# sleep3r/crispy

Hardware: AMD Instinct MI355X
Metric: concurrent real-time 48 kHz streams/GPU (RNNoise) (higher is better)
Workload: dtype f32; 1 GPU; Batched RNNoise: 4096 concurrent 48 kHz mono streams per GPU x 100 frames per step (BASELINE configs[1]), seeded synthetic int8 weights; streams_per_gpu=4096, output_finite=True

## Files before the change

crispy_amd/csrc/rn_kernels.hip:

```cpp
#include <type_traits>
#include "rn_common.h"
#include "rn_wave_sums.h"

namespace crispy {
namespace {

constexpr int WAVE = 64;

#ifdef RN_PROFILE
#define RN_PROF_DECL long long tprev_ = clock64(); \
  float* profp_ = (DBG && a.dbg) ? a.dbg + (long)blockIdx.x * RN_DBG_FLOATS + 3824 : nullptr;
#define STAMP(k) { const long long tn_ = clock64(); if (profp_ && threadIdx.x == 0) profp_[k] += (float)(tn_ - tprev_); tprev_ = tn_; }
#elif defined(RN_STOP_AFTER)
#define RN_PROF_DECL
#define STAMP(k) { if ((k) == RN_STOP_AFTER) { __syncthreads(); continue; } }
#else
#define RN_PROF_DECL
#define STAMP(k)
#endif

__device__ __constant__ int c_second_check[16] = {0, 0, 3, 2, 3, 2, 5, 2, 3, 2, 3, 2, 5, 2, 3, 2};

__device__ __forceinline__ float2 cmul(float2 a, float2 b) {
  return make_float2(a.x * b.x - a.y * b.y, a.x * b.y + a.y * b.x);
}
__device__ __forceinline__ float2 cadd(float2 a, float2 b) { return make_float2(a.x + b.x, a.y + b.y); }
__device__ __forceinline__ float2 csub(float2 a, float2 b) { return make_float2(a.x - b.x, a.y - b.y); }
__device__ __forceinline__ float2 cconj(float2 a) { return make_float2(a.x, -a.y); }

template <int CTRL, int ROW_MASK = 0xf>
__device__ __forceinline__ float dpp_mov(float v) {
  const int iv = __float_as_int(v);
  return __int_as_float(__builtin_amdgcn_update_dpp(0, iv, CTRL, ROW_MASK, 0xf, false));
}
template <int CTRL>
__device__ __forceinline__ float dpp_add(float v) {
  float r = v + dpp_mov<CTRL>(v);
  asm volatile("" : "+v"(r));
  return r;
}
template <class V>
__device__ __forceinline__ void lane_put(V& v, V s, int l) {
  static_assert(sizeof(V) == 4, "one dword");
  asm("v_writelane_b32 %0, %1, %2" : "+v"(v) : "s"(s), "n"(l));
}
template <class T>
__device__ __forceinline__ T ld_u32(const T* __restrict__ base, unsigned idx) {
  return *reinterpret_cast<const T*>(reinterpret_cast<const char*>(base) + idx * (unsigned)sizeof(T));
}
__device__ __forceinline__ float wave_sum(float v) {
  v += dpp_mov<0xB1>(v);
  v += dpp_mov<0x4E>(v);
  v += dpp_mov<0x141>(v);
  v += dpp_mov<0x140>(v);
  v += dpp_mov<0x142, 0xa>(v);
  v += dpp_mov<0x143, 0xc>(v);
  return __int_as_float(__builtin_amdgcn_readlane(__float_as_int(v), 63));
}

template <int NW>
__device__ __forceinline__ void rn_sync() {
  if constexpr (NW == 1) {
    __syncthreads();
  } else {
    __builtin_amdgcn_fence(__ATOMIC_RELEASE, "wavefront");
    __builtin_amdgcn_s_waitcnt(0xc07f);
    __builtin_amdgcn_wave_barrier();
    __builtin_amdgcn_fence(__ATOMIC_ACQUIRE, "wavefront");
  }
}

template <int R>
__device__ __forceinline__ void butterfly(const float2 (&v)[R], float2 (&o)[R]);

template <>
__device__ __forceinline__ void butterfly<4>(const float2 (&v)[4], float2 (&o)[4]) {
  const float2 s0 = cadd(v[0], v[2]), d0 = csub(v[0], v[2]);
  const float2 s1 = cadd(v[1], v[3]), d1 = csub(v[1], v[3]);
  o[0] = cadd(s0, s1);
  o[2] = csub(s0, s1);
  o[1] = make_float2(d0.x + d1.y, d0.y - d1.x);
  o[3] = make_float2(d0.x - d1.y, d0.y + d1.x);
}
template <>
// ... 318 lines not shown
      const int pidx = lane + WAVE * m;
      if (pidx < 200 && (lane & 1) == 0) { part[pidx >> 1] = clo[m]; part[100 + (pidx >> 1)] = chi[m]; }
    }
    band_total(Cout);
    if (XE) {
#pragma unroll
      for (int m = 0; m < 4; ++m) {
        const int pidx = lane + WAVE * m;
        if (pidx < 200 && (lane & 1) == 0) { part[pidx >> 1] = xlo[m]; part[100 + (pidx >> 1)] = xhi[m]; }
      }
      band_total(Xout);
    }
  }
}

struct TansigTab {
  float t[4];
  __device__ __forceinline__ void load(const float* __restrict__ table, int lane) {
#pragma unroll
    for (int q = 0; q < 4; ++q) t[q] = ld_u32(table, (unsigned)min(64 * q + lane, 200));
  }
  __device__ __forceinline__ float at(int i) const {
    const int addr = (i & 63) << 2;
    const float v0 = __int_as_float(__builtin_amdgcn_ds_bpermute(addr, __float_as_int(t[0])));
    const float v1 = __int_as_float(__builtin_amdgcn_ds_bpermute(addr, __float_as_int(t[1])));
    const float v2 = __int_as_float(__builtin_amdgcn_ds_bpermute(addr, __float_as_int(t[2])));
    const float v3 = __int_as_float(__builtin_amdgcn_ds_bpermute(addr, __float_as_int(t[3])));
    const int q = i >> 6;
    return q == 0 ? v0 : (q == 1 ? v1 : (q == 2 ? v2 : v3));
  }
};
__device__ __forceinline__ float tansig_approx(float x, const TansigTab& table) {
#pragma clang fp contract(off)
  const float x0 = x;
  float sign = 1.f;
  if (x < 0.f) { x = -x; sign = -1.f; }
  x = fminf(x, 8.f);
  const int i = (int)floorf(.5f + 25.f * x);
  x = x - .04f * (float)i;
  float y = table.at(i);
  const float dy = 1.f - y * y;
  y = y + (x * dy) * (1.f - y * x);
  y = sign * y;
  if (!(x0 > -8.f)) y = -1.f;
  if (!(x0 < 8.f)) y = 1.f;
  return y;
}
__device__ __forceinline__ float sigmoid_approx(float x, const TansigTab& table) {
  return .5f + .5f * tansig_approx(.5f * x, table);
}

typedef _Float16 h8 __attribute__((ext_vector_type(8)));
#define RN_LANE_RANGE(site) __builtin_assume((unsigned)lane < (unsigned)WAVE)
constexpr int RN_BLK3 = 1, RN_BLK2 = 1, RN_BLK1 = 4;

typedef unsigned int rn_u4 __attribute__((ext_vector_type(4)));
__device__ __forceinline__ float dot_vad(__amdgpu_buffer_rsrc_t rs, int w_off, const float* x, float acc0) {
  float acc = acc0, acc1 = 0.f;
#pragma unroll
  for (int k = 0; k < 3; ++k) {
    const h8 w = __builtin_bit_cast(h8, __builtin_amdgcn_raw_buffer_load_b128(rs, 0, (w_off + k) * 16, 0));
#pragma unroll
    for (int e = 0; e < 8; e += 2) {
      acc = fmaf((float)w[e], x[8 * k + e], acc);
      acc1 = fmaf((float)w[e + 1], x[8 * k + e + 1], acc1);
    }
  }
  return acc + acc1;
}

typedef int rn_i4 __attribute__((ext_vector_type(4)));
constexpr int RN_IMG8_LD = 144;
__device__ __forceinline__ float wave_max(float v) {
  unsigned u = __float_as_uint(v);
  auto dm = [](unsigned x, auto ctrl) {
    return (unsigned)__builtin_amdgcn_update_dpp(0, (int)x, decltype(ctrl)::value, 0xf, 0xf, false);
  };
  u = max(u, dm(u, std::integral_constant<int, 0xB1>{}));
  u = max(u, dm(u, std::integral_constant<int, 0x4E>{}));
  u = max(u, dm(u, std::integral_constant<int, 0x141>{}));
  u = max(u, dm(u, std::integral_constant<int, 0x140>{}));
  unsigned m = (unsigned)__builtin_amdgcn_readlane((int)u, 0);
  m = max(m, (unsigned)__builtin_amdgcn_readlane((int)u, 16));
  m = max(m, (unsigned)__builtin_amdgcn_readlane((int)u, 32));
  m = max(m, (unsigned)__builtin_amdgcn_readlane((int)u, 48));
  return __uint_as_float(m);
}
struct RnScale { float up, dn; };
__device__ __forceinline__ RnScale scale_of(float m) {
  int eb = (__float_as_int(m) >> 23) & 0xff;
  eb = min(max(eb, 64), 250);
  RnScale r;
  r.up = __int_as_float((283 - eb) << 23);
  r.dn = __int_as_float((eb - 29) << 23);
  return r;
}
__device__ __forceinline__ void digits_store(signed char* img, int i, float v, float up) {
  const int q = __float2int_rn(v * up);
  const unsigned r = ((unsigned)q + 0x00808080u) ^ 0x00808080u;
  img[i] = (signed char)(r & 0xff);
  img[RN_IMG8_LD + i] = (signed char)((r >> 8) & 0xff);
  img[2 * RN_IMG8_LD + i] = (signed char)((r >> 16) & 0xff);
  img[3 * RN_IMG8_LD + i] = (signed char)(r >> 24);
}
template <int NPAD, class F>
__device__ __forceinline__ RnScale image_i8(signed char* img, int lane, F f) {
  constexpr int NT = (NPAD + WAVE - 1) / WAVE;
  float v[NT];
  float m = 0.f;
#pragma unroll
  for (int j = 0; j < NT; ++j) {
    const int i = lane + WAVE * j;
    v[j] = i < NPAD ? f(min(i, NPAD - 1)) : 0.f;
    m = __uint_as_float(max(__float_as_uint(m), __float_as_uint(v[j]) & 0x7fffffffu));
  }
  const RnScale sc = scale_of(wave_max(m));
#pragma unroll
  for (int j = 0; j < NT; ++j) {
    const int i = lane + WAVE * j;
    if (i < NPAD) digits_store(img, i, v[j], sc.up);
  }
  return sc;
}
__device__ __forceinline__ rn_u4 wload8(__amdgpu_buffer_rsrc_t rs, int row16, int off16) {
  return __builtin_amdgcn_raw_buffer_load_b128(rs, row16, off16 * 16, 0);
}
template <int MK16, int NK16, int ROWS, int NR>
__device__ __forceinline__ void dotn_i(__amdgpu_buffer_rsrc_t rs, int w_off, int u_off, const int (&row)[NR],
                                       const signed char* xa, const signed char* xb, int toff, float sa, float sb,
                                       float (&acc)[NR]) {
  constexpr int K16 = MK16 + NK16;
  constexpr int BLK = NR >= 3 ? RN_BLK3 : (NR == 2 ? RN_BLK2 : RN_BLK1);
  constexpr int NBLK = (K16 + BLK - 1) / BLK;
  constexpr int NC = NR >= 3 ? 1 : 2;
  int row16[NR];
#pragma unroll
  for (int r = 0; r < NR; ++r) row16[r] = row[r] * 16;
  asm volatile("" : "+v"(toff));
  const rn_u4* xa4 = reinterpret_cast<const rn_u4*>(xa + toff);
  const rn_u4* xb4 = reinterpret_cast<const rn_u4*>(xb + toff);
  rn_u4 w[2][BLK][NR];
  rn_u4 xc = MK16 > 0 ? xa4[0] : xb4[0], xn = xc;
#pragma unroll
  for (int q = 0; q < BLK; ++q)
    if (q < K16) {
#pragma unroll
      for (int r = 0; r < NR; ++r)
        w[0][q][r] = wload8(rs, row16[r], q < MK16 ? w_off + q * ROWS : u_off + (q - MK16) * ROWS);
    }
  rn_i4 a4[NR][NC];
#pragma unroll
  for (int r = 0; r < NR; ++r)
#pragma unroll
    for (int c = 0; c < NC; ++c) a4[r][c] = rn_i4{0, 0, 0, 0};
  auto fold = [&](float s) {
#pragma unroll
    for (int r = 0; r < NR; ++r) {
      rn_i4 d = a4[r][0];
      if (NC == 2) d += a4[r][1];
      float f = (float)d[0] * s;
      f = fmaf((float)d[1], s * 256.f, f);
      f = fmaf((float)d[2], s * 65536.f, f);
      f = fmaf((float)d[3], s * 16777216.f, f);
      acc[r] += f;
#pragma unroll
      for (int c = 0; c < NC; ++c) a4[r][c] = rn_i4{0, 0, 0, 0};
    }
  };
#pragma unroll
  for (int blk = 0; blk < NBLK; ++blk) {
    if (blk + 1 < NBLK) {
#pragma unroll
      for (int q = 0; q < BLK; ++q) {
        const int k = (blk + 1) * BLK + q;
        if (k < K16) {
#pragma unroll
          for (int r = 0; r < NR; ++r)
            w[(blk + 1) & 1][q][r] = wload8(rs, row16[r], k < MK16 ? w_off + k * ROWS : u_off + (k - MK16) * ROWS);
        }
      }
    }
    __builtin_amdgcn_sched_barrier(0);
#pragma unroll
    for (int q = 0; q < BLK; ++q) {
      const int k = blk * BLK + q;
      if (k < K16) {
        if (k + 1 < K16) xn = k + 1 < MK16 ? xa4[k + 1] : xb4[k + 1 - MK16];
        if (MK16 > 0 && NK16 > 0 && k == MK16) fold(sa);
        if (!(k == 0 || (MK16 > 0 && NK16 > 0 && k == MK16))) {
#pragma unroll
          for (int r = 0; r < NR; ++r)
#pragma unroll
            for (int c = 0; c < NC; ++c) asm volatile("" : "+v"(a4[r][c]));
        }
        __builtin_amdgcn_sched_barrier(0);
#pragma unroll
        for (int e = 0; e < 4; ++e) {
#pragma unroll
          for (int r = 0; r < NR; ++r)
            a4[r][e % NC] = __builtin_amdgcn_mfma_i32_4x4x4i8((int)xc[e], (int)w[blk & 1][q][r][e], a4[r][e % NC], 0, 0, 0);
        }
        __builtin_amdgcn_sched_barrier(0);
        xc = xn;
      }
    }
  }
  fold(NK16 > 0 ? sb : sa);
}
template <int K16, int ROWS>
__device__ __forceinline__ float dot_i(__amdgpu_buffer_rsrc_t rs, int w_off, int row, const signed char* x, int toff,
                                       float s, float acc0) {
  const int rows[1] = {row};
  float acc[1] = {acc0};
  dotn_i<K16, 0, ROWS, 1>(rs, w_off, w_off, rows, x, x, toff, s, s, acc);
  return acc[0];
}
template <int NW, int M, int N>
__device__ __forceinline__ void gru_layer_i(__amdgpu_buffer_rsrc_t rs, int w_off, int u_off,
                                            const float* __restrict__ bias, const signed char* in_img, float sin,
                                            float* state, float* zbuf, signed char* st_img, int toff,
                                            const TansigTab& tansig, int lane) {
  constexpr int ROWS = 3 * N;
  constexpr int MK16 = (M + 15) / 16, NK16 = (N + 15) / 16;
  constexpr int NRZ = (2 * N + WAVE - 1) / WAVE, NRC = (N + WAVE - 1) / WAVE;
  const float S = 1.f / 256.f;
  const RnScale sst = image_i8<NK16 * 16>(st_img, lane, [&](int i) { return i < N ? state[min(i, N - 1)] : 0.f; });
  rn_sync<NW>();
  {
    int rows[NRZ];
    float acc[NRZ];
#pragma unroll
    for (int r = 0; r < NRZ; ++r) {
      rows[r] = min(lane + WAVE * r, 2 * N - 1);
      acc[r] = ld_u32(bias, (unsigned)rows[r]);
    }
    dotn_i<MK16, NK16, ROWS, NRZ>(rs, w_off, u_off, rows, in_img, st_img, toff, sin, sst.dn, acc);
#pragma unroll
    for (int r = 0; r < NRZ; ++r) {
      const int row = lane + WAVE * r;
      const float s = sigmoid_approx(S * acc[r], tansig);
      if (row < 2 * N) {
        if (row < N) zbuf[row] = s;
        else digits_store(st_img, row - N, state[row - N] * s, sst.up);
      }
    }
  }
  rn_sync<NW>();
  {
    int rows[NRC];
    float acc[NRC];
#pragma unroll
    for (int r = 0; r < NRC; ++r) {
      rows[r] = 2 * N + min(lane + WAVE * r, N - 1);
      acc[r] = ld_u32(bias, (unsigned)rows[r]);
    }
    dotn_i<MK16, NK16, ROWS, NRC>(rs, w_off, u_off, rows, in_img, st_img, toff, sin, sst.dn, acc);
#pragma unroll
    for (int r = 0; r < NRC; ++r) {
      const int i = lane + WAVE * r;
      if (i < N) {
        float c = S * acc[r];
        c = c < 0.f ? 0.f : c;
        const float z = zbuf[i];
        state[i] = z * state[i] + (1.f - z) * c;
      }
    }
  }
  rn_sync<NW>();
}

struct alignas(16) RnSlot {
  float2 A[482];
  float2 Bb[482];
  float U[200];
  float Ex[24], Ep[24], Exp[24];
  int pitch_index;
  float pitch_gain;
  int silence;
  int pad;
};
template <int NW> struct RnLdsT;
template <> struct alignas(16) RnLdsT<1> {
  RnSlot s[1];
  float ceps[8 * 22];
  float rnn_state[168];
};
template <> struct alignas(16) RnLdsT<3> {
  RnSlot s[2];
  float2 pa[482];
  float2 pb[482];
  float ceps[8 * 22];
  float rnn_state[168];
  int pitch_index[2];
  float pitch_gain[2];
};
static_assert(sizeof(RnLdsT<1>) <= 10240, "16 workgroups per CU need <= 10 KB of LDS each");
static_assert(6 * sizeof(RnLdsT<3>) <= 160 * 1024, "six stage-pipelined streams per CU");

constexpr int U_G = 0, U_R = 24, U_VAD = 46, U_LY = 48;
constexpr int PL_FEAT = 800, PL_Z = 842, PL_DENSE = 938, PL_A_FREE = 800, PL_U_FREE = 48;

struct Cand {
  float num, den;
  int idx;
};
__device__ __forceinline__ bool cand_better(const Cand& a, const Cand& b) {
  const float l = a.num * b.den, r = b.num * a.den;
  return (l > r) || (!(r > l) && a.idx < b.idx);
}
__device__ __forceinline__ Cand wave_best(Cand c) {
#pragma unroll
  for (int off = 32; off > 0; off >>= 1) {
    Cand o;
    o.num = __shfl_xor(c.num, off, WAVE);
    o.den = __shfl_xor(c.den, off, WAVE);
    o.idx = __shfl_xor(c.idx, off, WAVE);
    if (cand_better(o, c)) c = o;
  }
  c.num = __shfl(c.num, 0, WAVE);
  c.den = __shfl(c.den, 0, WAVE);
  c.idx = __shfl(c.idx, 0, WAVE);
  return c;
}

typedef float rn_f2 __attribute__((ext_vector_type(2)));
__device__ __forceinline__ void lag_window(const float* xr, int lane, float (&xv)[8]) {
#pragma unroll
  for (int m = 0; m < 7; ++m) xv[m] = xr[WAVE * m];
  xv[7] = 0.f;
  if (lane < 32) xv[7] = xr[WAVE * 7];
}
template <int NL, bool SQ>
__device__ __forceinline__ void lag_dots(const float (&xv)[8], const float* const (&yr)[NL], int lane, float (&sxy)[NL],
                                         float (&syy)[NL]) {
#pragma unroll
  for (int q = 0; q < NL; ++q) { sxy[q] = 0.f; syy[q] = 0.f; }
#pragma unroll
  for (int q = 0; q < NL; ++q) {
#pragma unroll
    for (int m = 0; m < 7; ++m) {
      const float y = yr[q][WAVE * m];
      sxy[q] = fmaf(xv[m], y, sxy[q]);
      if (SQ) syy[q] = fmaf(y, y, syy[q]);
    }
  }
  if (lane < 32) {
#pragma unroll
    for (int q = 0; q < NL; ++q) {
      const float y = yr[q][WAVE * 7];
      sxy[q] = fmaf(xv[7], y, sxy[q]);
      if (SQ) syy[q] = fmaf(y, y, syy[q]);
    }
  }
  wave_sums<NL>(sxy);
  if (SQ) wave_sums<NL>(syy);
}

#ifndef RN_POISON_LDS
#define RN_POISON_LDS 0
#endif
[[maybe_unused]] __device__ __forceinline__ void rn_poison_lds(uint32_t* p, int words) {
  for (int i = threadIdx.x; i < words; i += WAVE) p[i] = 0x7fc0dead;
  __syncthreads();
}

__device__ __forceinline__ float2* rn_lds_lp(RnLdsT<1>& L) { return L.s[0].Bb; }
__device__ __forceinline__ float2* rn_lds_sa(RnLdsT<1>& L) { return L.s[0].A; }
__device__ __forceinline__ float2* rn_lds_lp(RnLdsT<3>& L) { return L.pb; }
__device__ __forceinline__ float2* rn_lds_sa(RnLdsT<3>& L) { return L.pa; }

template <bool DBG, int NW>
__device__ __forceinline__ void rn_frame_body(const RnArgs& a) {
  __shared__ RnLdsT<NW> L;
  const int wave = NW == 1 ? 0 : (int)(threadIdx.x >> 6);
  const int lane0 = threadIdx.x & (WAVE - 1);
  const int b = blockIdx.x;
  if (b >= a.B) return;
  int lane = lane0;
  const RnTables* tab = a.tab;
  const float* xs = a.xhp + (long)b * a.xhp_stride;
  if constexpr (NW == 1) {
    unsigned hw;
    asm volatile("s_getreg_b32 %0, hwreg(HW_REG_HW_ID)" : "=s"(hw));
    const unsigned pr = hw & 3u;
    if (pr == 0) __builtin_amdgcn_s_setprio(0);
    else if (pr == 1) __builtin_amdgcn_s_setprio(1);
    else if (pr == 2) __builtin_amdgcn_s_setprio(2);
    else __builtin_amdgcn_s_setprio(3);
  }

#if RN_POISON_LDS
  rn_poison_lds(reinterpret_cast<uint32_t*>(&L), sizeof(L) / 4);
#endif

  const bool own_a = NW == 1 || wave == 0, own_b = NW == 1 || wave == 1, own_c = NW == 1 || wave == 2;
  if (own_b)
    for (int i = lane; i < 176; i += WAVE) L.ceps[i] = a.ceps[(long)b * 176 + i];
  if (own_c)
    for (int i = lane; i < 168; i += WAVE) L.rnn_state[i] = a.rnn[(long)b * 168 + i];
  float2 synth[4];
  float* synth_g = a.synth + (long)b * 480;
#pragma unroll
  for (int m = 0; m < 4; ++m) {
    const int n = lane + WAVE * m;
// ... 120 lines not shown
        float y[14];
  #pragma unroll
        for (int q = 0; q < 14; ++q) {
          float sum = w[q + 5];
          sum = fmaf(lpc2[0], w[q + 4], sum);
          sum = fmaf(lpc2[1], w[q + 3], sum);
          sum = fmaf(lpc2[2], w[q + 2], sum);
          sum = fmaf(lpc2[3], w[q + 1], sum);
          sum = fmaf(lpc2[4], w[q], sum);
          y[q] = sum;
        }
        rn_sync<NW>();
  #pragma unroll
        for (int q = 0; q < 14; ++q)
          if (base + q < 864) lp[base + q] = y[q];
        rn_sync<NW>();
      }
      STAMP(0)
      lane = lane0;
      asm volatile("" : "+v"(lane));
      RN_LANE_RANGE(4);

      float* x4 = Sa;
      float* y4 = Sa + 240;
      float* pre = Sa;
      {
        float vx[4], vy[7];
  #pragma unroll
        for (int m = 0; m < 4; ++m) vx[m] = lp[384 + 2 * min(lane + WAVE * m, 239)];
  #pragma unroll
        for (int m = 0; m < 7; ++m) vy[m] = lp[2 * min(lane + WAVE * m, 386)];
  #pragma unroll
        for (int m = 0; m < 4; ++m) {
          const int j = lane + WAVE * m;
          if (j < 240) x4[j] = vx[m];
        }
  #pragma unroll
        for (int m = 0; m < 7; ++m) {
          const int j = lane + WAVE * m;
          if (j < 392) y4[j] = j < 387 ? vy[m] : 0.f;
        }
      }
      rn_sync<NW>();
      int best0, best1;
      {
        float xc[3] = {0.f, 0.f, 0.f};
        {
          const float4* xv4 = reinterpret_cast<const float4*>(x4);
          const float* yp = y4 + 3 * min(lane, 48);
          float y0 = yp[0], y1 = yp[1];
  #pragma unroll 4
          for (int j4 = 0; j4 < 60; ++j4) {
            const float4 xv = xv4[j4];
            const int j = 4 * j4;
            const float y2 = yp[j + 2], y3 = yp[j + 3], y4v = yp[j + 4], y5 = yp[j + 5];
            xc[0] = fmaf(xv.x, y0, xc[0]);
            xc[1] = fmaf(xv.x, y1, xc[1]);
            xc[2] = fmaf(xv.x, y2, xc[2]);
            xc[0] = fmaf(xv.y, y1, xc[0]);
            xc[1] = fmaf(xv.y, y2, xc[1]);
            xc[2] = fmaf(xv.y, y3, xc[2]);
            xc[0] = fmaf(xv.z, y2, xc[0]);
            xc[1] = fmaf(xv.z, y3, xc[1]);
            xc[2] = fmaf(xv.z, y4v, xc[2]);
            xc[0] = fmaf(xv.w, y3, xc[0]);
            xc[1] = fmaf(xv.w, y4v, xc[1]);
            xc[2] = fmaf(xv.w, y5, xc[2]);
            y0 = y4v;
            y1 = y5;
          }
        }
        STAMP(1)
        {
          float loc[7];
          float run = 0.f;
  #pragma unroll
          for (int q = 0; q < 7; ++q) {
            const int j = 7 * lane + q;
            const float v = j < 392 ? y4[j] : 0.f;
            loc[q] = run;
            run = fmaf(v, v, run);
          }
          float incl = run;
  #pragma unroll
          for (int off = 1; off < WAVE; off <<= 1) {
            const float o = __shfl_up(incl, off, WAVE);
            if (lane >= off) incl += o;
          }
          const float excl = incl - run;
          rn_sync<NW>();
  #pragma unroll
          for (int q = 0; q < 7; ++q)
            if (7 * lane + q < 392) pre[7 * lane + q] = excl + loc[q];
        }
        rn_sync<NW>();
        Cand c0 = {-1.f, 0.f, 1 << 20}, c1 = {-1.f, 0.f, 1 << 20};
        int nvalid = 0;
  #pragma unroll
        for (int rr = 0; rr < 3; ++rr) {
          const int lag = 3 * lane + rr;
          if (lag < 147 && xc[rr] > 0.f) {
            const float syy = fmaxf(1.f, 1.f + (pre[lag + 240] - pre[lag]));
            const float x16 = xc[rr] * 1e-12f;
            const Cand c = {x16 * x16, syy, lag};
            ++nvalid;
            if (cand_better(c, c0)) { c1 = c0; c0 = c; }
            else if (cand_better(c, c1)) c1 = c;
          }
        }
        const int total_valid = __popcll(__ballot(nvalid > 0)) == 0 ? 0 : (int)wave_sum((float)nvalid);
        const Cand w0 = wave_best(c0);
        const Cand mine = (c0.idx == w0.idx) ? c1 : c0;
        const Cand w1 = wave_best(mine);
        if (total_valid == 0) { best0 = 0; best1 = 1; }
        else if (total_valid == 1) { best0 = w0.idx; best1 = 0; }
        else { best0 = w0.idx; best1 = w1.idx; }
      }
      best0 = __builtin_amdgcn_readfirstlane(best0);
      best1 = __builtin_amdgcn_readfirstlane(best1);
      rn_sync<NW>();
      STAMP(2)

      float* fine = Sa;
      float xwin[8];
      for (int i = lane; i < 296; i += WAVE) fine[i] = 0.f;
      rn_sync<NW>();
      {
        const int ca = 2 * min(best0, best1), cb = 2 * max(best0, best1);
        Cand bestc = {-1.f, 0.f, 0};
        bool any = false;
        int lagi[10];
        bool use[10];
        const float* yr[10];
  #pragma unroll
        for (int q = 0; q < 10; ++q) {
          const int pass = q / 5, d = q % 5 - 2;
          const int i = (pass == 0 ? ca : cb) + d;
          use[q] = !(i < 0 || i >= 294) && !(pass == 1 && abs(i - ca) <= 2);
          lagi[q] = use[q] ? i : 0;
          yr[q] = lp + lagi[q] + lane;
        }
        float sxy[10], syy[10];
        lag_window(lp + 384 + lane, lane, xwin);
        lag_dots<10, true>(xwin, yr, lane, sxy, syy);
  #pragma unroll
        for (int q = 0; q < 10; ++q) {
          if (use[q]) {
            const float syq = fmaxf(1.f, 1.f + syy[q]);
            const float xv = fmaxf(-1.f, sxy[q]);
            if (lane == 0) fine[lagi[q]] = xv;
            if (xv > 0.f) {
              const float x16 = xv * 1e-12f;
              const Cand c = {x16 * x16, syq, lagi[q]};
              if (!any || cand_better(c, bestc)) { bestc = c; any = true; }
            }
          }
        }
        rn_sync<NW>();
        const int bp = any ? bestc.idx : 0;
        int offset = 0;
        if (bp > 0 && bp < 293) {
          const float fa = fine[bp - 1], fb = fine[bp], fc = fine[bp + 1];
          if ((fc - fa) > .7f * (fb - fa)) offset = 1;
          else if ((fa - fc) > .7f * (fb - fc)) offset = -1;
        }
        pitch_index = __builtin_amdgcn_readfirstlane(768 - (2 * bp - offset));
      }
      rn_sync<NW>();
      STAMP(3)
      if (DBG && a.dbg && t == a.T - 1) {
        float* D = a.dbg + (long)b * RN_DBG_FLOATS;
        for (int i = lane; i < 864; i += WAVE) D[984 + i] = lp[i];
        if (lane == 0) D[1848] = (float)pitch_index;
  #ifndef RN_PROFILE
        for (int i = lane; i < 480; i += WAVE) D[3824 + i] = xw[480 + i];
  #endif
      }

      {
        const float* x = lp + 384;
        int T0 = pitch_index / 2;
        const int prev_period = last_period / 2;
        if (T0 >= 384) T0 = 383;
        int T = T0;
        float xx, xy;
        {
          const float* yr[2] = {x + lane, x - T0 + lane};
          float sa[2], sb[2];
          lag_dots<2, false>(xwin, yr, lane, sa, sb);
          xx = sa[0];
          xy = sa[1];
        }
        float* yyl = Sa + 296;
        {
          float loc[6];
          float run = 0.f;
  #pragma unroll
          for (int q = 0; q < 6; ++q) {
            const int m = 6 * lane + 1 + q;
            const float u = x[-m], v = x[480 - m];
            run += u * u - v * v;
            loc[q] = run;
          }
          float incl = run;
  #pragma unroll
          for (int off = 1; off < WAVE; off <<= 1) {
            const float o = __shfl_up(incl, off, WAVE);
            if (lane >= off) incl += o;
          }
          const float excl = incl - run;
  #pragma unroll
          for (int q = 0; q < 6; ++q) yyl[6 * lane + 1 + q] = fmaxf(0.f, xx + (excl + loc[q]));
          if (lane == 0) yyl[0] = xx;
        }
        rn_sync<NW>();
        float yy = yyl[T0];
        float best_xy = xy, best_yy = yy;
        const float g0 = xy / sqrtf(1.f + xx * yy);
        float g = g0;
        int t1v = 0, t1bv = 0;
        float xya = 0.f, xyb = 0.f;
        static_assert((2 * 383 + 14) / (2 * 14) < 30, "candidates k >= 14 are out of range for every T0");
  #pragma unroll
        for (int c = 0; c < 3; ++c) {
          const int k0 = 2 + 4 * c;
          if ((2 * T0 + k0) / (2 * k0) >= 30) {
            constexpr int NKC = 4;
            const float* yr[2 * NKC];
            int t1[NKC], t1b[NKC];
  #pragma unroll
            for (int q = 0; q < NKC; ++q) {
              const int k = k0 + q;
              t1[q] = 0; t1b[q] = 0;
              const int T1 = (2 * T0 + k) / (2 * k);
              if (T1 >= 30) {
                t1[q] = T1;
                if (k == 2) t1b[q] = (T1 + T0 > 384) ? T0 : T0 + T1;
                else t1b[q] = (2 * c_second_check[k] * T0 + k) / (2 * k);
              }
              yr[2 * q] = x - t1[q] + lane;
              yr[2 * q + 1] = x - t1b[q] + lane;
            }
            float sa[2 * NKC], sb[2 * NKC];
            lag_dots<2 * NKC, false>(xwin, yr, lane, sa, sb);
  #pragma unroll
            for (int q = 0; q < NKC; ++q) {
              const int l = k0 + q - 2;
              lane_put(t1v, t1[q], l);
              lane_put(t1bv, t1b[q], l);
              lane_put(xya, sa[2 * q], l);
              lane_put(xyb, sa[2 * q + 1], l);
            }
          }
        }
        {
          const int T1 = t1v;
          const float xyk = .5f * (xya + xyb);
          const float yyk = .5f * (yyl[t1v] + yyl[t1bv]);
          const int k = lane + 2;
          const float g1 = xyk / sqrtf(1.f + xx * yyk);
          float cont;
          if (abs(T1 - prev_period) <= 1) cont = last_gain;
          else if (abs(T1 - prev_period) <= 2 && 5 * k * k < T0) cont = .5f * last_gain;
          else cont = 0.f;
          float thresh = fmaxf(.3f, .7f * g0 - cont);
          if (T1 < 90) thresh = fmaxf(.4f, .85f * g0 - cont);
          else if (T1 < 60) thresh = fmaxf(.5f, .9f * g0 - cont);
          const unsigned long long pass = __ballot(lane < 14 && T1 >= 30 && g1 > thresh);
          if (pass != 0ull) {
            const int w = 63 - __builtin_clzll(pass);
            best_xy = __int_as_float(__builtin_amdgcn_readlane(__float_as_int(xyk), w));
            best_yy = __int_as_float(__builtin_amdgcn_readlane(__float_as_int(yyk), w));
            T = __builtin_amdgcn_readlane(T1, w);
            g = __int_as_float(__builtin_amdgcn_readlane(__float_as_int(g1), w));
          }
        }
        best_xy = fmaxf(0.f, best_xy);
        float pgv = (best_yy <= best_xy) ? 1.f : best_xy / (best_yy + 1.f);
        float xc3[3];
        {
          const float* yr[3] = {x - (T - 1) + lane, x - T + lane, x - (T + 1) + lane};
          float sb[3];
          lag_dots<3, false>(xwin, yr, lane, xc3, sb);
        }
        int offset = 0;
        if ((xc3[2] - xc3[0]) > .7f * (xc3[1] - xc3[0])) offset = 1;
        else if ((xc3[0] - xc3[2]) > .7f * (xc3[1] - xc3[2])) offset = -1;
        if (pgv > g) pgv = g;
        pitch_index = 2 * T + offset;
        if (pitch_index < 60) pitch_index = 60;
// ... 82 lines not shown
        }
      }
      {
        if (lane < 6) {
          float v = se * dct_norm;
          if (lane == 0) v -= 1.3f;
          if (lane == 1) v -= 0.9f;
          Rb[KB_FEAT + 34 + lane] = v;
        }
        if (lane == 6) Rb[KB_FEAT + 40] = .01f * (float)(pitch_index - 300);
        silence = E < 0.04f;
        if (!silence && lane < RN_NB) {
          float v = sl * dct_norm;
          if (lane == 0) v -= 12.f;
          if (lane == 1) v -= 4.f;
          Rb[KB_FEAT + lane] = v;
          L.ceps[memid * RN_NB + lane] = v;
        }
      }
      rn_sync<NW>();
      if (silence) {
        if (lane < RN_NFEAT) Rb[KB_FEAT + lane] = 0.f;
        if (lane < RN_NB) SL.U[U_G + lane] = 0.f;
        rn_sync<NW>();
      } else {
        {
          const int m1 = (memid < 1) ? 8 + memid - 1 : memid - 1;
          const int m2 = (memid < 2) ? 8 + memid - 2 : memid - 2;
          if (lane < 6) {
            const float c0 = L.ceps[memid * RN_NB + lane];
            const float c1 = L.ceps[m1 * RN_NB + lane];
            const float c2 = L.ceps[m2 * RN_NB + lane];
            Rb[KB_FEAT + lane] = c0 + c1 + c2;
            Rb[KB_FEAT + RN_NB + lane] = c0 - c2;
            Rb[KB_FEAT + RN_NB + 6 + lane] = c0 - 2.f * c1 + c2;
          }
          memid = (memid + 1 == 8) ? 0 : memid + 1;
        }
        {
          const int ci = lane >> 3, cj = lane & 7;
          float dist = 0.f;
  #pragma unroll
          for (int k = 0; k < RN_NB; ++k) {
            const float d = L.ceps[ci * RN_NB + k] - L.ceps[cj * RN_NB + k];
            dist = fmaf(d, d, dist);
          }
          float md = (ci == cj) ? 1e15f : dist;
          md = fminf(md, dpp_mov<0xB1>(md));
          md = fminf(md, dpp_mov<0x4E>(md));
          md = fminf(md, dpp_mov<0x141>(md));
          const float sv = wave_sum(md) * .125f;
          if (lane == 0) Rb[KB_FEAT + 41] = sv / 8.f - 2.1f;
        }
        rn_sync<NW>();
        STAMP(7)
      }
      if constexpr (NW > 1) {
        if (lane == 0) { SL.pitch_index = pitch_index; SL.pitch_gain = pitch_gain; SL.silence = silence ? 1 : 0; }
      }
    }
    if (own_c) {
      if constexpr (NW > 1) {
        pitch_index = __builtin_amdgcn_readfirstlane(SL.pitch_index);
        pitch_gain = SL.pitch_gain;
        silence = __builtin_amdgcn_readfirstlane(SL.silence) != 0;
      }
      if (!silence) {
        lane = lane0;
        asm volatile("" : "+v"(lane));
        RN_LANE_RANGE(1);
        const float S = 1.f / 256.f;
        float* feat = Rb + KB_FEAT;
        float* dense = Rb + PL_DENSE;
        float* zbuf = Rb + PL_Z;
        TansigTab tansig;
        tansig.load(tab->tansig, lane);
        signed char* in_img = reinterpret_cast<signed char*>(SL.U + PL_U_FREE);
        signed char* st_img = reinterpret_cast<signed char*>(Xf + PL_A_FREE);
        const int toff = (lane & 3) * RN_IMG8_LD;
        RnScale sc = image_i8<48>(in_img, lane, [&](int i) { return i < RN_NFEAT ? feat[i] : 0.f; });
        rn_sync<NW>();
        {
          const int row = min(lane, 23);
          const float acc = dot_i<rn_k16(42), 24>(wrs, RnPack8::ID_W, row, in_img, toff, sc.dn, wpf[RnPack::ID_B + row]);
          const float d = tansig_approx(S * acc, tansig);
          if (lane < 24) dense[lane] = d;
        }
        rn_sync<NW>();
        sc = image_i8<32>(in_img, lane, [&](int i) { return i < 24 ? dense[i] : 0.f; });
        gru_layer_i<NW, 24, 24>(wrs, RnPack8::VG_W, RnPack8::VG_R, wpf + RnPack::VG_B, in_img, sc.dn,
                            L.rnn_state, zbuf, st_img, toff, tansig, lane);
        {
          float acc = 0.f;
          if (lane == 0) {
            acc = wpf[RnPack::VO_B];
            acc = dot_vad(wrs, RnPack::VO_W, L.rnn_state, acc);
          }
          const float v = sigmoid_approx(S * acc, tansig);
          if (lane == 0) SL.U[U_VAD] = v;
        }
        sc = image_i8<96>(in_img, lane, [&](int i) {
          return i < 24 ? dense[i] : (i < 48 ? L.rnn_state[i - 24] : (i < 90 ? feat[i - 48] : 0.f)); });
        rn_sync<NW>();
        vad_prob = SL.U[U_VAD];
        STAMP(8)
        gru_layer_i<NW, 90, 48>(wrs, RnPack8::NG_W, RnPack8::NG_R, wpf + RnPack::NG_B, in_img, sc.dn,
                            L.rnn_state + 24, zbuf, st_img, toff, tansig, lane);
        STAMP(9)
        sc = image_i8<128>(in_img, lane, [&](int i) { return i < 72 ? L.rnn_state[i] : (i < 114 ? feat[i - 72] : 0.f); });
        rn_sync<NW>();
        gru_layer_i<NW, 114, 96>(wrs, RnPack8::DG_W, RnPack8::DG_R, wpf + RnPack::DG_B, in_img, sc.dn,
                             L.rnn_state + 72, zbuf, st_img, toff, tansig, lane);
        sc = image_i8<96>(st_img, lane, [&](int i) { return L.rnn_state[72 + i]; });
        rn_sync<NW>();
        {
          const int row = min(lane, RN_NB - 1);
          const float acc = dot_i<rn_k16(96), RN_NB>(wrs, RnPack8::DO_W, row, st_img, toff, sc.dn, wpf[RnPack::DO_B + row]);
          const float gv = sigmoid_approx(S * acc, tansig);
          if (lane < RN_NB) SL.U[U_G + lane] = gv;
        }
        rn_sync<NW>();
        STAMP(10)

        lane = lane0;
        asm volatile("" : "+v"(lane));
        RN_LANE_RANGE(2);
        float2 fq[4];
        int bq[4];
        {
          float4 pq[4];
  #pragma unroll
          for (int m = 0; m < 4; ++m) {
            const unsigned pidx = (unsigned)min(lane + WAVE * m, 199);
            pq[m] = *reinterpret_cast<const float4*>(SL.Bb + 2 * pidx);
            fq[m] = ld_u32(reinterpret_cast<const float2*>(tab->bin_frac), pidx);
            bq[m] = ld_u32(tab->bin_band, 2 * pidx);
          }
          if (lane < RN_NB) {
            const float ex = SL.Exp[lane], gg = SL.U[U_G + lane];
            float r;
            if (ex > gg) r = 1.f;
            else r = (ex * ex) * (1.f - gg * gg) / (.001f + (gg * gg) * (1.f - ex * ex));
            r = sqrtf(fminf(1.f, fmaxf(0.f, r)));
            r *= sqrtf(SL.Ex[lane] / (1e-8f + SL.Ep[lane]));
            SL.U[U_R + lane] = r;
          }
          rn_sync<NW>();
          float* part = Xf + PL_A_FREE;
          float* part_hi = SL.U + PL_U_FREE;
  #pragma unroll
          for (int m = 0; m < 4; ++m) {
            const int pidx = lane + WAVE * m;
            if (pidx < 200) {
              const float r0 = SL.U[U_R + bq[m]], r1 = SL.U[U_R + bq[m] + 1];
              const float rf0 = (1.f - fq[m].x) * r0 + fq[m].x * r1;
              const float rf1 = (1.f - fq[m].y) * r0 + fq[m].y * r1;
              float4 x = *reinterpret_cast<const float4*>(SL.A + 2 * pidx);
              x.x = fmaf(rf0, pq[m].x, x.x);
              x.y = fmaf(rf0, pq[m].y, x.y);
              x.z = fmaf(rf1, pq[m].z, x.z);
              x.w = fmaf(rf1, pq[m].w, x.w);
              *reinterpret_cast<float4*>(SL.A + 2 * pidx) = x;
              float e0 = x.x * x.x; e0 += x.y * x.y;
              float e1 = x.z * x.z; e1 += x.w * x.w;
              float lo = (1.f - fq[m].x) * e0 + (1.f - fq[m].y) * e1;
              float hi = fq[m].x * e0 + fq[m].y * e1;
              lo = dpp_add<0xB1>(lo);
              hi = dpp_add<0xB1>(hi);
              if ((lane & 1) == 0) { part[pidx >> 1] = lo; part_hi[pidx >> 1] = hi; }
            }
          }
        }
        rn_sync<NW>();
        float sum;
        {
          const float* part = Xf + PL_A_FREE;
          const float* part_hi = SL.U + PL_U_FREE;
          sum = band_sum(part, part_hi, be, lane);
        }
        if (lane < RN_NB) {
          SL.U[U_R + lane] = sqrtf(SL.Ex[lane] / (1e-8f + sum));
          const float gg = fmaxf(SL.U[U_G + lane], .6f * lastg);
          SL.U[U_G + lane] = gg;
          lastg = gg;
        }
        rn_sync<NW>();
        float nq[4][2], gq[4][2];
        float4 xq[4];
  #pragma unroll
        for (int m = 0; m < 4; ++m) {
          nq[m][0] = SL.U[U_R + bq[m]]; nq[m][1] = SL.U[U_R + bq[m] + 1];
          gq[m][0] = SL.U[U_G + bq[m]]; gq[m][1] = SL.U[U_G + bq[m] + 1];
          xq[m] = *reinterpret_cast<const float4*>(SL.A + 2 * min(lane + WAVE * m, 199));
        }
  #pragma unroll
        for (int m = 0; m < 4; ++m) {
          const int pidx = lane + WAVE * m;
          if (pidx < 200) {
            const float n0 = nq[m][0], n1 = nq[m][1];
            const float g0 = gq[m][0], g1 = gq[m][1];
// ... 136 lines not shown
```

Measured before the change: 751,800 concurrent real-time 48 kHz streams (whole job).

## Pin scale math to scalar regs, use swizzle/bpermute reductions, branchless candidate select

Moves the quantization scale computation into a header and uses inline asm to keep it in scalar registers. Power-of-two scale multiplies become exponent-bit adds. The candidate argmax reduction is rewritten with ds_bpermute/ds_swizzle, branchless selection and readlane broadcasts, and the prefix scans use bpermute in place of __shfl_up. The number of MFMA accumulator chains is now parameterized by wave count (one chain when NW==1), which cuts accumulator registers but lengthens the dependency chain.

```diff
diff --git a/crispy_amd/csrc/rn_kernels.hip b/crispy_amd/csrc/rn_kernels.hip
--- a/crispy_amd/csrc/rn_kernels.hip
+++ b/crispy_amd/csrc/rn_kernels.hip
@@ -1,5 +1,6 @@
 #include <type_traits>
 #include "rn_common.h"
+#include "rn_scale.h"
 #include "rn_wave_sums.h"
 
 namespace crispy {
@@ -484,18 +485,11 @@
   u = max(u, dm(u, std::integral_constant<int, 0x140>{}));
   unsigned m = (unsigned)__builtin_amdgcn_readlane((int)u, 0);
   m = max(m, (unsigned)__builtin_amdgcn_readlane((int)u, 16));
+  asm volatile("" : "+s"(m));
   m = max(m, (unsigned)__builtin_amdgcn_readlane((int)u, 32));
+  asm volatile("" : "+s"(m));
   m = max(m, (unsigned)__builtin_amdgcn_readlane((int)u, 48));
   return __uint_as_float(m);
-}
-struct RnScale { float up, dn; };
-__device__ __forceinline__ RnScale scale_of(float m) {
-  int eb = (__float_as_int(m) >> 23) & 0xff;
-  eb = min(max(eb, 64), 250);
-  RnScale r;
-  r.up = __int_as_float((283 - eb) << 23);
-  r.dn = __int_as_float((eb - 29) << 23);
-  return r;
 }
 __device__ __forceinline__ void digits_store(signed char* img, int i, float v, float up) {
   const int q = __float2int_rn(v * up);
@@ -527,14 +521,15 @@
 __device__ __forceinline__ rn_u4 wload8(__amdgpu_buffer_rsrc_t rs, int row16, int off16) {
   return __builtin_amdgcn_raw_buffer_load_b128(rs, row16, off16 * 16, 0);
 }
-template <int MK16, int NK16, int ROWS, int NR>
+constexpr int rn_chains(int nw) { return nw == 1 ? 1 : 2; }
+template <int MK16, int NK16, int ROWS, int NR, int NCH>
 __device__ __forceinline__ void dotn_i(__amdgpu_buffer_rsrc_t rs, int w_off, int u_off, const int (&row)[NR],
                                        const signed char* xa, const signed char* xb, int toff, float sa, float sb,
                                        float (&acc)[NR]) {
   constexpr int K16 = MK16 + NK16;
   constexpr int BLK = NR >= 3 ? RN_BLK3 : (NR == 2 ? RN_BLK2 : RN_BLK1);
   constexpr int NBLK = (K16 + BLK - 1) / BLK;
-  constexpr int NC = NR >= 3 ? 1 : 2;
+  constexpr int NC = NR >= 3 ? 1 : NCH;
   int row16[NR];
 #pragma unroll
   for (int r = 0; r < NR; ++r) row16[r] = row[r] * 16;
@@ -561,9 +556,9 @@
       rn_i4 d = a4[r][0];
       if (NC == 2) d += a4[r][1];
       float f = (float)d[0] * s;
-      f = fmaf((float)d[1], s * 256.f, f);
-      f = fmaf((float)d[2], s * 65536.f, f);
-      f = fmaf((float)d[3], s * 16777216.f, f);
+      f = fmaf((float)d[1], scale_shift<8>(s), f);
+      f = fmaf((float)d[2], scale_shift<16>(s), f);
+      f = fmaf((float)d[3], scale_shift<24>(s), f);
       acc[r] += f;
 #pragma unroll
       for (int c = 0; c < NC; ++c) a4[r][c] = rn_i4{0, 0, 0, 0};
@@ -609,12 +604,12 @@
   }
   fold(NK16 > 0 ? sb : sa);
 }
-template <int K16, int ROWS>
+template <int K16, int ROWS, int NCH>
 __device__ __forceinline__ float dot_i(__amdgpu_buffer_rsrc_t rs, int w_off, int row, const signed char* x, int toff,
                                        float s, float acc0) {
   const int rows[1] = {row};
   float acc[1] = {acc0};
-  dotn_i<K16, 0, ROWS, 1>(rs, w_off, w_off, rows, x, x, toff, s, s, acc);
+  dotn_i<K16, 0, ROWS, 1, NCH>(rs, w_off, w_off, rows, x, x, toff, s, s, acc);
   return acc[0];
 }
 template <int NW, int M, int N>
@@ -636,7 +631,7 @@
       rows[r] = min(lane + WAVE * r, 2 * N - 1);
       acc[r] = ld_u32(bias, (unsigned)rows[r]);
     }
-    dotn_i<MK16, NK16, ROWS, NRZ>(rs, w_off, u_off, rows, in_img, st_img, toff, sin, sst.dn, acc);
+    dotn_i<MK16, NK16, ROWS, NRZ, rn_chains(NW)>(rs, w_off, u_off, rows, in_img, st_img, toff, sin, sst.dn, acc);
 #pragma unroll
     for (int r = 0; r < NRZ; ++r) {
       const int row = lane + WAVE * r;
@@ -656,7 +651,7 @@
       rows[r] = 2 * N + min(lane + WAVE * r, N - 1);
       acc[r] = ld_u32(bias, (unsigned)rows[r]);
     }
-    dotn_i<MK16, NK16, ROWS, NRC>(rs, w_off, u_off, rows, in_img, st_img, toff, sin, sst.dn, acc);
+    dotn_i<MK16, NK16, ROWS, NRC, rn_chains(NW)>(rs, w_off, u_off, rows, in_img, st_img, toff, sin, sst.dn, acc);
 #pragma unroll
     for (int r = 0; r < NRC; ++r) {
       const int i = lane + WAVE * r;
@@ -702,26 +697,46 @@
 constexpr int U_G = 0, U_R = 24, U_VAD = 46, U_LY = 48;
 constexpr int PL_FEAT = 800, PL_Z = 842, PL_DENSE = 938, PL_A_FREE = 800, PL_U_FREE = 48;
 
+__device__ __forceinline__ float lane_up(float v, int lane4, int off) {
+  return __int_as_float(__builtin_amdgcn_ds_bpermute(lane4 + 4 * (WAVE - off), __float_as_int(v)));
+}
+
 struct Cand {
   float num, den;
   int idx;
 };
 __device__ __forceinline__ bool cand_better(const Cand& a, const Cand& b) {
   const float l = a.num * b.den, r = b.num * a.den;
-  return (l > r) || (!(r > l) && a.idx < b.idx);
-}
-__device__ __forceinline__ Cand wave_best(Cand c) {
-#pragma unroll
-  for (int off = 32; off > 0; off >>= 1) {
-    Cand o;
-    o.num = __shfl_xor(c.num, off, WAVE);
-    o.den = __shfl_xor(c.den, off, WAVE);
-    o.idx = __shfl_xor(c.idx, off, WAVE);
-    if (cand_better(o, c)) c = o;
-  }
-  c.num = __shfl(c.num, 0, WAVE);
-  c.den = __shfl(c.den, 0, WAVE);
-  c.idx = __shfl(c.idx, 0, WAVE);
+  const bool gt = l > r, ngt = !(r > l), lt = a.idx < b.idx;
+  return gt | (ngt & lt);
+}
+__device__ __forceinline__ Cand cand_pick(bool take_a, const Cand& a, const Cand& b) {
+  return Cand{take_a ? a.num : b.num, take_a ? a.den : b.den, take_a ? a.idx : b.idx};
+}
+template <int OFF>
+__device__ __forceinline__ int lane_xor(int v) {
+  return __builtin_amdgcn_ds_swizzle(v, (OFF << 10) | 0x1f);
+}
+template <int OFF>
+__device__ __forceinline__ Cand cand_xor(const Cand& c) {
+  return Cand{__int_as_float(lane_xor<OFF>(__float_as_int(c.num))), __int_as_float(lane_xor<OFF>(__float_as_int(c.den))),
+              lane_xor<OFF>(c.idx)};
+}
+__device__ __forceinline__ Cand wave_best(Cand c, int half_addr) {
+  {
+    const Cand o = {__int_as_float(__builtin_amdgcn_ds_bpermute(half_addr, __float_as_int(c.num))),
+                    __int_as_float(__builtin_amdgcn_ds_bpermute(half_addr, __float_as_int(c.den))),
+                    __builtin_amdgcn_ds_bpermute(half_addr, c.idx)};
+    c = cand_pick(cand_better(o, c), o, c);
+  }
+  { const Cand o = cand_xor<16>(c); c = cand_pick(cand_better(o, c), o, c); }
+  { const Cand o = cand_xor<8>(c); c = cand_pick(cand_better(o, c), o, c); }
+  { const Cand o = cand_xor<4>(c); c = cand_pick(cand_better(o, c), o, c); }
+  { const Cand o = cand_xor<2>(c); c = cand_pick(cand_better(o, c), o, c); }
+  { const Cand o = cand_xor<1>(c); c = cand_pick(cand_better(o, c), o, c); }
+  c.num = __int_as_float(__builtin_amdgcn_readlane(__float_as_int(c.num), 0));
+  c.den = __int_as_float(__builtin_amdgcn_readlane(__float_as_int(c.den), 0));
+  c.idx = __builtin_amdgcn_readlane(c.idx, 0);
   return c;
 }
 
@@ -1008,9 +1023,10 @@
             run = fmaf(v, v, run);
           }
           float incl = run;
+          const int up_addr = lane << 2;
   #pragma unroll
           for (int off = 1; off < WAVE; off <<= 1) {
-            const float o = __shfl_up(incl, off, WAVE);
+            const float o = lane_up(incl, up_addr, off);
             if (lane >= off) incl += o;
           }
           const float excl = incl - run;
@@ -1024,26 +1040,25 @@
         int nvalid = 0;
   #pragma unroll
         for (int rr = 0; rr < 3; ++rr) {
-          const int lag = 3 * lane + rr;
-          if (lag < 147 && xc[rr] > 0.f) {
-            const float syy = fmaxf(1.f, 1.f + (pre[lag + 240] - pre[lag]));
-            const float x16 = xc[rr] * 1e-12f;
-            const Cand c = {x16 * x16, syy, lag};
-            ++nvalid;
-            if (cand_better(c, c0)) { c1 = c0; c0 = c; }
-            else if (cand_better(c, c1)) c1 = c;
-          }
+          const int lag = 3 * lane + rr, lagc = 3 * min(lane, 48) + rr;
+          const bool valid = lag < 147 && xc[rr] > 0.f;
+          const float syy = fmaxf(1.f, 1.f + (pre[lagc + 240] - pre[lagc]));
+          const float x16 = xc[rr] * 1e-12f;
+          const Cand c = {x16 * x16, syy, lag};
+          nvalid += valid ? 1 : 0;
+          const bool b0 = valid & cand_better(c, c0), b1 = valid & cand_better(c, c1);
+          c1 = cand_pick(b0, c0, cand_pick(b1, c, c1));
+          c0 = cand_pick(b0, c, c0);
         }
         const int total_valid = __popcll(__ballot(nvalid > 0)) == 0 ? 0 : (int)wave_sum((float)nvalid);
-        const Cand w0 = wave_best(c0);
+        const int half_addr = (lane ^ 32) << 2;
+        const Cand w0 = wave_best(c0, half_addr);
         const Cand mine = (c0.idx == w0.idx) ? c1 : c0;
-        const Cand w1 = wave_best(mine);
+        const Cand w1 = wave_best(mine, half_addr);
         if (total_valid == 0) { best0 = 0; best1 = 1; }
         else if (total_valid == 1) { best0 = w0.idx; best1 = 0; }
         else { best0 = w0.idx; best1 = w1.idx; }
       }
-      best0 = __builtin_amdgcn_readfirstlane(best0);
-      best1 = __builtin_amdgcn_readfirstlane(best1);
       rn_sync<NW>();
       STAMP(2)
 
@@ -1129,9 +1144,10 @@
             loc[q] = run;
           }
           float incl = run;
+          const int up_addr = lane << 2;
   #pragma unroll
           for (int off = 1; off < WAVE; off <<= 1) {
-            const float o = __shfl_up(incl, off, WAVE);
+            const float o = lane_up(incl, up_addr, off);
             if (lane >= off) incl += o;
           }
           const float excl = incl - run;
@@ -1380,7 +1396,7 @@
         rn_sync<NW>();
         {
           const int row = min(lane, 23);
-          const float acc = dot_i<rn_k16(42), 24>(wrs, RnPack8::ID_W, row, in_img, toff, sc.dn, wpf[RnPack::ID_B + row]);
+          const float acc = dot_i<rn_k16(42), 24, rn_chains(NW)>(wrs, RnPack8::ID_W, row, in_img, toff, sc.dn, wpf[RnPack::ID_B + row]);
           const float d = tansig_approx(S * acc, tansig);
           if (lane < 24) dense[lane] = d;
         }
@@ -1413,7 +1429,7 @@
         rn_sync<NW>();
         {
           const int row = min(lane, RN_NB - 1);
-          const float acc = dot_i<rn_k16(96), RN_NB>(wrs, RnPack8::DO_W, row, st_img, toff, sc.dn, wpf[RnPack::DO_B + row]);
+          const float acc = dot_i<rn_k16(96), RN_NB, rn_chains(NW)>(wrs, RnPack8::DO_W, row, st_img, toff, sc.dn, wpf[RnPack::DO_B + row]);
           const float gv = sigmoid_approx(S * acc, tansig);
           if (lane < RN_NB) SL.U[U_G + lane] = gv;
         }
diff --git a/crispy_amd/csrc/rn_scale.h b/crispy_amd/csrc/rn_scale.h
--- /dev/null
+++ b/crispy_amd/csrc/rn_scale.h
@@ -0,0 +1,36 @@
+#pragma once
+
+#if defined(__HIP_DEVICE_COMPILE__)
+#define RN_SCALE_FN __device__ __forceinline__
+#define RN_PIN_SCALAR(x) asm volatile("" : "+s"(x))
+#define RN_PIN_SCALAR2(x, y) asm volatile("" : "+s"(x), "+s"(y))
+#elif defined(__HIPCC__)
+#define RN_SCALE_FN __device__ __forceinline__
+#define RN_PIN_SCALAR(x) ((void)0)
+#define RN_PIN_SCALAR2(x, y) ((void)0)
+#else
+#define RN_SCALE_FN inline
+#define RN_PIN_SCALAR(x) ((void)0)
+#define RN_PIN_SCALAR2(x, y) ((void)0)
+#endif
+
+namespace crispy {
+
+struct RnScale { float up, dn; };
+RN_SCALE_FN RnScale scale_of(float m) {
+  int mi = __builtin_bit_cast(int, m);
+  RN_PIN_SCALAR(mi);
+  int eb = (mi >> 23) & 0xff;
+  eb = eb > 64 ? eb : 64;
+  RN_PIN_SCALAR(eb);
+  eb = eb < 250 ? eb : 250;
+  int up = (283 - eb) << 23, dn = (eb - 29) << 23;
+  RN_PIN_SCALAR2(up, dn);
+  return RnScale{__builtin_bit_cast(float, up), __builtin_bit_cast(float, dn)};
+}
+template <int E>
+RN_SCALE_FN float scale_shift(float s) {
+  return __builtin_bit_cast(float, __builtin_bit_cast(int, s) + (E << 23));
+}
+
+}
```

After: 763,300 concurrent real-time 48 kHz streams (whole job), median of 6. 1.5% higher.
